# Ignaciagothe/tda-eeg-audio

Hardware: AMD Instinct MI355X
Metric: windows/sec end-to-end (dist->Rips H0/H1->Wasserstein), 47-ch EEG (higher is better)
Workload: dtype f64; 1 GPU; configs[4]+configs[2]: 1416 recordings x 5 bands x 15 selected windows = 106200 (EEG 47x250 f64, audio 250 f64) window pairs per pass, the whole job; per pair corr->dist->Rips H0/H1 (EEG 47 pts), tau per recording-band, Takens dim 3 sub 2 + Rips (audio, 23..123 pts over the bands), Wasserstein H0+H1, features, per-recording reductions; one all-gather of the (1416, 5x48) rows per pass; windows_per_pass=106200, windows_per_gpu_per_pass=106200, input_bytes_per_gpu=10195200000, batches_per_pass=1, windows_per_batch=106200, parallelism=recordings dealt over 1 rank(s), one all-gather per pass, batches_in_flight=3, hip_graph=True, batches_rerun_with_full_ladder=0

## Files before the change

### tda_eeg_audio_amd/csrc/rips.hip

```cpp
#include "common.h"
#include "corr_dist_dev.h"
#include <stdlib.h>

#ifndef CLOUD_NB
#define CLOUD_NB 8192
#endif
#ifndef NARROW_NT
#define NARROW_NT 512
#endif
#ifndef NARROW_WAVES
#define NARROW_WAVES 6
#endif
#if defined(TDA_PROFILE) && !defined(TDA_PROFILE_STOPS_ONLY)
#define NARROW_NB (NARROW_NT == 384 ? 1536 : 1024)
#else
#define NARROW_NB (NARROW_NT == 384 ? 1536 : 2048)
#endif
#define NARROW_EMAX 7626
#define NT_MAX 512
#define RANK_NONE 0x7fffu

#ifdef TDA_PROFILE
__device__ unsigned long long g_prof[48];
#ifdef TDA_PROFILE_STOPS_ONLY
#define PROF_BEGIN() do {} while (0)
#define PROF_RESUME() do {} while (0)
#define PROF_MARK(i) do {} while (0)
#define PROF_COUNT(i, v) do {} while (0)
#define PROF_FLUSH() do {} while (0)
#else
__shared__ unsigned long long prof_lds[48];
#define PROF_BEGIN()                                                       \
    if (threadIdx.x < 48) prof_lds[threadIdx.x] = 0ull;                    \
    __syncthreads();                                                       \
    unsigned long long prof_t0 = clock64()
#define PROF_RESUME() unsigned long long prof_t0 = clock64()
#define PROF_MARK(i)                                                       \
    do {                                                                   \
        unsigned long long prof_t1 = clock64();                            \
        if (threadIdx.x == 0) prof_lds[i] += prof_t1 - prof_t0;            \
        prof_t0 = prof_t1;                                                 \
// ... 95 lines not shown

__device__ __forceinline__ int edge_row(int e)
{
    const int a = (int)((1.0f + __builtin_amdgcn_sqrtf(1.0f + 8.0f * (float)e)) * 0.5f);
    const int t = tri2(a);
    return a + (t + a <= e ? 1 : 0) - (t > e ? 1 : 0);
}

#ifndef TDA_NO_EDGE_TABLE
struct EdgeTable {
    u16 v[8192 + 512];
    constexpr EdgeTable() : v()
    {
        int a = 1, b = 0;
        for (int e = 0; e < 8192 + 512; ++e) { v[e] = (u16)((a << 8) | b); if (++b == a) { ++a; b = 0; } }
    }
};
__device__ const EdgeTable g_edge_ab = EdgeTable();
__device__ __forceinline__ u32 edge_ab(int e) { return (u32)g_edge_ab.v[e]; }
#else
__device__ __forceinline__ u32 edge_ab(int e) { const int a = edge_row(e); return (u32)((a << 8) | (e - tri2(a))); }
#endif

struct WgVote {
    u32* slots;
    int parity;
};
template <int NT>
__device__ __forceinline__ bool wg_any(WgVote& v, bool p)
{
    static_assert(NT % 64 == 0 && NT <= 512, "slots are read as one or two 16-byte words; slots beyond NT / 64 hold zero");
    const bool w = __ballot(p) != 0ull;
    u32* s = v.slots + 8 * v.parity;
    if ((threadIdx.x & 63) == 0) s[threadIdx.x >> 6] = w ? 1u : 0u;
    __syncthreads();
    v.parity ^= 1;
    const uint4 x = *reinterpret_cast<const uint4*>(s);
    u32 r = x.x | x.y | x.z | x.w;
    if (NT > 256) { const uint4 y = *reinterpret_cast<const uint4*>(s + 4); r |= y.x | y.y | y.z | y.w; }
    return r != 0u;
}
template <int NT>
__device__ __forceinline__ bool wg_all(WgVote& v, bool p) { return !wg_any<NT>(v, !p); }

__device__ __forceinline__ int wave_incl_scan_i32(int v)
{
#define TDA_DPP_ADD_(CTRL, RM) v += __builtin_amdgcn_update_dpp(0, v, CTRL, RM, 0xF, true)
    TDA_DPP_ADD_(0x111, 0xF);
    TDA_DPP_ADD_(0x112, 0xF);
    TDA_DPP_ADD_(0x114, 0xF);
    TDA_DPP_ADD_(0x118, 0xF);
    TDA_DPP_ADD_(0x142, 0xA);
    TDA_DPP_ADD_(0x143, 0xC);
#undef TDA_DPP_ADD_
    return v;
}

// ... 289 lines not shown
    return __syncthreads_or(bad ? 1 : 0) ? TDA_WIN_LDS_GUARD : 0;
}
#else
#define GUARD_BYTES 0
__device__ __forceinline__ void guard_write(unsigned char*, const RipsLayout&) {}
__device__ __forceinline__ int guard_check(unsigned char*, const RipsLayout&) { return 0; }
#endif

#define MISC_COMP 0
#define MISC_CAND 512
#define MISC_WV (512 + 128)
#define MISC_MIN (512 + 192)
#define MISC_DONE (512 + 208)
#define MISC_SORTCNT (512 + 224)
#define MISC_SHARED (MISC_DONE + NT_MAX)
#define MISC_CKEY (MISC_SHARED + 96)
#define MISC_LIST MISC_CKEY
#define MISC_LIST_BYTES (4 * NT_MAX + 1280)
#define MISC_ADJ (MISC_LIST + MISC_LIST_BYTES)
#define MISC_ADJC (MISC_ADJ + 128 * 16)
#define MISC_BRANK (MISC_ADJC + 128 * 16)
#define MISC_BYTES(ncls) (MISC_BRANK + 8 * (ncls))

template <int NT, int NVW, int W, typename WT, bool NARROW, class KEYFN>
__device__ __forceinline__ void rips_sweep(int n, int E, int Ev, const u16* rank, const u16* ord, Psi<W, WT>* psi, int psi_bytes,
                           unsigned char* misc, KEYFN keyfn, double* h0, int h0_cap, double* h1, int h1_cap,
                           int& out_k0, int& out_k1, int& out_status)
{
    static_assert(!NARROW || W == 1, "the narrow layout is the point-cloud first pass");
    int psi_cap = 0;
    const int tid0 = threadIdx.x;
    const int lane0 = tid0 & 63, wave = uni(tid0 >> 6);
    int* brank = reinterpret_cast<int*>(misc + MISC_BRANK);
    u64* cand = reinterpret_cast<u64*>(misc + MISC_CAND);
    unsigned char* done = misc + MISC_DONE;
    SweepShared* shared = reinterpret_cast<SweepShared*>(misc + MISC_SHARED);
    u64* adj = reinterpret_cast<u64*>(misc + MISC_ADJ);
    constexpr int WB = 8 * (int)sizeof(WT);
    float* bkey = reinterpret_cast<float*>(misc + MISC_BRANK + 4 * WB * W);
    u64* adjc = reinterpret_cast<u64*>(misc + MISC_ADJC);

    if constexpr (!NARROW) for (int e = tid0; e < E; e += NT) psi[e] = pzero<W, WT>();
    for (int i = tid0; i < WB * W; i += NT) { brank[i] = -1; bkey[i] = 0.f; }
    for (int i = tid0; i < 256; i += NT) { adj[i] = 0ull; adjc[i] = 0ull; }
    if (tid0 == 0) {
        u32* lc = reinterpret_cast<u32*>(misc + MISC_MIN);
        lc[0] = 0u; lc[1] = 0xffffffffu; lc[2] = 0u;
        lc[3] = 0u;
        shared->status = 0;
    }
    if (tid0 < 16) {
        reinterpret_cast<u32*>(misc + MISC_WV)[tid0] = 0u;
        cand[tid0] = 0ull;
    }
    __syncthreads();

    WgVote vote{reinterpret_cast<u32*>(misc + MISC_WV), 0};
    WT alive[W];
#pragma unroll
    for (int c = 0; c < W; ++c) alive[c] = 0;
    int k0 = 0, k1 = 0, merges = 0, status = 0;
    int compA = lane0, compB = lane0 + 64;

    int clen = NT;
    int ordcls = 0;
    int cov_next = tid0;
#ifdef TDA_PROFILE
    int prof_rneed = 0, prof_chunk = -1;
#endif
    PROF_RESUME();
    for (int r0 = 0; r0 < Ev && !status; r0 += clen) {
        int tid = tid0;
        LAUNDER(tid);
        const int lane = tid & 63;
        clen = NT;
        PROF_MARK(15);
#ifdef TDA_PROFILE
        ++prof_chunk;
#endif
        PROF_COUNT(23, 1);
        const int r = r0 + tid;
        const bool valid = r < Ev;
        int a = 1, b = 0;
        if (valid) { const u32 pk = ord[r]; a = (int)(pk >> 8); b = (int)(pk & 255u); }
        const int tab = tri2(a) + b;
        const int slot = NARROW ? r : tab;
        if constexpr (NARROW) {
            psi_cap = (psi_bytes - 2 * (E - r0)) >> 2;
            if (r < psi_cap) psi[r] = pzero<W, WT>();
        }
        u64 M[NVW], M0[NVW];
        u64 Aj[NVW], Bj[NVW];
#pragma unroll
        for (int w = 0; w < NVW; ++w) { M[w] = 0; M0[w] = 0; Aj[w] = 0; Bj[w] = 0; }
        if (valid) {
#pragma unroll
            for (int w = 0; w < NVW; ++w) { Aj[w] = adj[2 * a + w]; Bj[w] = adj[2 * b + w]; M0[w] = Aj[w] & Bj[w]; }
        }
        {
            volatile u32* turn = reinterpret_cast<volatile u32*>(misc + MISC_MIN) + 2;
            if (wave > 0) {
                int trips = 0;
                for (;;) {
                    const u32 t = (u32)uni((int)*turn);
                    if (t >= (u32)wave) break;
                    if (++trips > TDA_POLL_LIMIT) { if (lane == 0) turn[1] = 1u; break; }
                    if (t + 1u < (u32)wave) __builtin_amdgcn_s_sleep(TDA_TURN_SLEEP); else __builtin_amdgcn_s_sleep(0);
                }
            }
            __builtin_amdgcn_fence(__ATOMIC_ACQUIRE, "workgroup");
            if (valid) {
#pragma unroll
                for (int w = 0; w < NVW; ++w) M[w] = (Aj[w] | adjc[2 * a + w]) & (Bj[w] | adjc[2 * b + w]);
                atomicOr(reinterpret_cast<unsigned long long*>(&adjc[2 * a + (b >> 6)]), 1ull << (b & 63));
                atomicOr(reinterpret_cast<unsigned long long*>(&adjc[2 * b + (a >> 6)]), 1ull << (a & 63));
            }
            LDS_ORDER();
            if (lane == 0 && !(TDA_FAULT(1) && wave == 3)) *turn = (u32)wave + 1u;
        }
        if (valid) {
            const int ta0 = tri2(a), tb0 = tri2(b);
#pragma unroll
            for (int w = 0; w < NVW; ++w) {
                u64 cc = (Aj[w] | adjc[2 * a + w]) & (Bj[w] | adjc[2 * b + w]) & ~M[w];
                while (cc) {
                    const int v0 = 64 * w + __builtin_ctzll(cc); cc &= cc - 1ull;
                    const bool ok1 = cc != 0ull; const int v1 = ok1 ? 64 * w + __builtin_ctzll(cc) : v0; cc &= cc - 1ull;
                    const int t0 = tri2(v0), t1 = tri2(v1);
                    const u32 xa0 = rank[v0 < a ? ta0 + v0 : t0 + a], xb0 = rank[v0 < b ? tb0 + v0 : t0 + b];
                    const u32 xa1 = rank[v1 < a ? ta0 + v1 : t1 + a], xb1 = rank[v1 < b ? tb0 + v1 : t1 + b];
                    if ((int)(xa0 > xb0 ? xa0 : xb0) < r) M[w] |= 1ull << (v0 & 63);
                    if (ok1 && (int)(xa1 > xb1 ? xa1 : xb1) < r) M[w] |= 1ull << (v1 & 63);
                }
            }
        }
        u64 many = 0;
#pragma unroll
        for (int w = 0; w < NVW; ++w) many |= M[w];
        const bool is_cand = valid && many == 0;
        int vstar = 0, d1 = 0, d2 = 0, q1 = 0, q2 = 0;
        {
            u64 many0 = 0;
#pragma unroll
            for (int w = 0; w < NVW; ++w) many0 |= M0[w];
            if (many0) {
                if (NVW == 1 || M0[0]) vstar = __builtin_ctzll(M0[0]);
                else vstar = 64 + __builtin_ctzll(M0[NVW - 1]);
            } else if (many) {
                if (NVW == 1 || M[0]) vstar = __builtin_ctzll(M[0]);
                else vstar = 64 + __builtin_ctzll(M[NVW - 1]);
            }
            if (valid && many != 0) {
                d1 = pair_index(a, vstar); d2 = pair_index(b, vstar);
                q1 = (int)rank[d1] - r0; q2 = (int)rank[d2] - r0;
                if (TDA_FAULT(2) && tid == 77 && q1 >= 0) q1 = tid;
            }
        }
        PROF_MARK(4);
        PROF_STOPC(11, out_k0 = k0; out_k1 = k1; out_status = 0);
        u64* mbal = reinterpret_cast<u64*>(misc + MISC_COMP);
        u64* zbal = mbal + 8;
        int* offs = reinterpret_cast<int*>(mbal + 16);
        u16* freebits = reinterpret_cast<u16*>(misc + MISC_CKEY);
        float mykey = 0.f;
        if (is_cand) mykey = keyfn(r, a, b);
        {
            const u64 bal = __ballot(is_cand), zb = __ballot(is_cand && mykey == 0.0f);
            if (lane == 0) { cand[wave] = bal; zbal[wave] = zb; }
        }
        done[tid] = 0;
        __syncthreads();
        PROF_MARK(21);
        PROF_STOPC(12, out_k0 = k0; out_k1 = k1; out_status = 0);
        int nfree = 0;
#pragma unroll
        for (int c = 0; c < W; ++c) nfree += __builtin_popcountll((u64)(WT)~alive[c]);
        int ncand = 0;
#pragma unroll
        for (int w = 0; w < NT / 64; ++w) ncand += __builtin_popcountll(cand[w]);
        int btot = 0;
        if (ncand > 0) {
// ... 152 lines not shown
        bool row = mrg && mykey != 0.0f;
        const u64 below = (1ull << lane) - 1ull;
        const int bpre = offs[wave] + __builtin_popcountll(__ballot(birth) & below);
        const int rpre = offs[8 + wave] + __builtin_popcountll(__ballot(row) & below);
        btot = uni(offs[16]);
        const int rtot = uni(offs[17]), mtot = uni(offs[18]);
        if (!status) {
            if (row) {
                const int pos = k0 + rpre;
                if (pos < h0_cap) { h0[2 * pos] = 0.0; h0[2 * pos + 1] = (double)mykey; }
            }
            k0 += rtot; merges += mtot;
            if (birth) {
                const int idx = (int)freebits[bpre];
                const int cw = idx / WB, bit = idx & (WB - 1);
                Psi<W, WT> nv = pzero<W, WT>();
#pragma unroll
                for (int c = 0; c < W; ++c)
                    if (c == cw) nv.w[c] = ((WT)1 << bit);
                if (!NARROW || r < psi_cap) psi[slot] = nv;
                brank[idx] = r;
                bkey[idx] = mykey;
            }
            if (W == 1 && wave == 0 && btot > 0) {
                const int nal = __builtin_popcountll((u64)alive[0]);
                if (lane >= nal && lane < nal + btot) ordcls = (int)freebits[lane - nal];
            }
            int left = btot;
#pragma unroll
            for (int c = 0; c < W; ++c) {
                const u64 f_ = (u64)(WT)~alive[c];
                const int pc = __builtin_popcountll(f_);
                if (left >= pc) { alive[c] = (WT)~(WT)0; left -= pc; }
                else if (left > 0) {
                    int lo = 0, hi = 63;
                    while (lo < hi) {
                        const int mid = (lo + hi) >> 1;
                        if (__builtin_popcountll(f_ & ((2ull << mid) - 1ull)) >= left) hi = mid; else lo = mid + 1;
                    }
                    alive[c] |= (WT)(f_ & ((2ull << lo) - 1ull));
                    left = 0;
                }
            }
        }
        }
        if (status) break;
        PROF_MARK(5);
// ... 194 lines not shown
                const u32 wmin = wave_min_u32_dpp(firstkey);
                if (lane == 0 && wmin != 0xffffffffu) atomicMin(&lcnt[1], wmin);
            }
            __syncthreads();
            PROF_MARK(17);
            PROF_STOPC(17, out_k0 = k0; out_k1 = k1; out_status = 0);
            const u32 cnt = (u32)uni((int)lcnt[0]);
            if (cnt == 0u) break;
            const bool complete = cnt <= (u32)LCAP;
            PROF_COUNT(11, 1);
            PROF_COUNT(12, cnt);
            if (!complete) {
                PROF_COUNT(13, 1);
                if (firstkey == lcnt[1]) {
                    *reinterpret_cast<u32*>(list) = firstkey;
#pragma unroll
                    for (int c = 0; c < W; ++c) *reinterpret_cast<WT*>(list + 4 + c * (int)sizeof(WT)) = firsty.w[c];
                }
                __syncthreads();
            }
            WT alive_before[W];
#pragma unroll
            for (int c = 0; c < W; ++c) alive_before[c] = alive[c];
            if (wave == 0) {
                TDA_SOLO_BEGIN();
                const int nl = complete ? (int)cnt : 1;
                u32 ek[LPL];
                Psi<W, WT> ev[LPL];
#pragma unroll
                for (int q = 0; q < LPL; ++q) {
                    const int idx = lane + 64 * q;
                    ek[q] = 0xffffffffu; ev[q] = pzero<W, WT>();
                    if (idx < nl) {
                        ek[q] = *reinterpret_cast<const u32*>(list + ES * idx);
#pragma unroll
                        for (int c = 0; c < W; ++c)
                            ev[q].w[c] = *reinterpret_cast<const WT*>(list + ES * idx + 4 + c * (int)sizeof(WT));
                    }
                }
                if (SORTED && complete) {
                    constexpr int HW = HISTN / 256;
                    u32* hw = reinterpret_cast<u32*>(hist) + HW * lane;
                    const u32 x0 = hw[0], x1 = HW == 2 ? hw[HW - 1] : 0u;
                    const u32 s0 = __builtin_amdgcn_sad_u8(x0, 0u, 0u);
                    const u32 tot = HW == 2 ? __builtin_amdgcn_sad_u8(x1, 0u, s0) : s0;
                    const u32 before = (u32)wave_incl_scan_i32((int)tot) - tot;
                    hw[0] = x0 * 0x01010101u - x0 + before * 0x01010101u;
// ... 163 lines not shown
                    for (int c = 0; c < W; ++c)
                        if (c == ycw) alive[c] &= (WT)~((WT)1 << ybit);
                    ++nk;
                }
                PROF_MARK(31);
                PROF_COUNT(10, nk);
                if (FTAB) {
                    const bool mine_ok = lane < nk;
                    float key = 0.f;
                    if (mine_ok) {
                        const u32 pkk = ord[(int)myrk];
                        key = keyfn((int)myrk, (int)(pkk >> 8), (int)(pkk & 255u));
                    }
                    const bool emit = mine_ok && key > mybirth;
                    const u64 bal = __ballot(emit);
                    const int pos = k1 + __builtin_popcountll(bal & ((1ull << lane) - 1ull));
                    if (emit && pos < h1_cap) { h1[2 * pos] = (double)mybirth; h1[2 * pos + 1] = (double)key; }
                    k1 += __builtin_popcountll(bal);
                    if (mine_ok) {
                        Psi<W, WT>* ftab = reinterpret_cast<Psi<W, WT>*>(list);
                        ftab[WB * (int)(mycode >> 8) + (int)(mycode & 255u)] = vimg;
                    }
                }
                if (lane == 0) {
#pragma unroll
                    for (int c = 0; c < W; ++c) shared->alive[c] = (u64)alive[c];
                    shared->k1 = k1; shared->nk = nk; shared->more = more; shared->status = status;
                }
                TDA_SOLO_END();
            }
            __syncthreads();
            PROF_MARK(18);
            PROF_STOPC(18, out_k0 = k0; out_k1 = k1; out_status = 0);
            WT kmask[W];
#pragma unroll
            for (int c = 0; c < W; ++c) {
                const WT na = sizeof(WT) == 8 ? (WT)uni64(shared->alive[c]) : (WT)uni((int)(u32)shared->alive[c]);
                kmask[c] = alive_before[c] & (WT)~na; alive[c] = na;
            }
            k1 = uni(shared->k1);
            const int nk = uni(shared->nk);
            const bool more = uni(shared->more) != 0;
            status = uni(shared->status);
            if (status) break;
            if (FTAB) {
                const Psi<W, WT>* ftab = reinterpret_cast<const Psi<W, WT>*>(list);
                const int seen_end = r0 + clen < Ev ? r0 + clen : Ev;
#pragma unroll 4
                for (int rr = tid; rr < seen_end; rr += NT) {
                    const int e = NARROW ? rr : edge_flat(ord[rr]);
                    const Psi<W, WT> p = psi[e];
                    WT anyh = 0;
#pragma unroll
                    for (int c = 0; c < W; ++c) anyh |= p.w[c] & kmask[c];
                    if (!anyh) continue;
                    Psi<W, WT> q;
#pragma unroll
                    for (int c = 0; c < W; ++c) q.w[c] = p.w[c] & (WT)~kmask[c];
#pragma unroll
                    for (int c = 0; c < W; ++c) {
                        u64 hh = (u64)(p.w[c] & kmask[c]);
                        while (hh) {
                            const int bit = __builtin_ctzll(hh);
                            hh &= hh - 1ull;
                            q = pxor(q, ftab[WB * c + bit]);
                        }
                    }
// ... 9 lines not shown
                        kc[j] = j0 + j < nk ? *reinterpret_cast<const u32*>(list + ES * jj) : 0xffffffffu;
#pragma unroll
                        for (int c = 0; c < W; ++c) kw[j].w[c] = *reinterpret_cast<const WT*>(list + ES * jj + 4 + c * (int)sizeof(WT));
                    }
#pragma unroll 4
                    for (int rr = tid; rr < (r0 + clen < Ev ? r0 + clen : Ev); rr += NT) {
                        const int e = NARROW ? rr : edge_flat(ord[rr]);
                        Psi<W, WT> p = psi[e];
                        bool changed = false;
#pragma unroll
                        for (int j = 0; j < 4; ++j) {
                            if (kc[j] == 0xffffffffu) continue;
                            const int jcw = (int)(kc[j] >> 8), jbit = (int)(kc[j] & 255u);
                            WT sel = 0;
#pragma unroll
                            for (int c = 0; c < W; ++c)
                                if (c == jcw) sel = (p.w[c] >> jbit) & (WT)1;
                            if (sel) { p = pxor(p, kw[j]); changed = true; }
                        }
                        if (changed) psi[e] = p;
                    }
                }
            }
            PROF_MARK(19);
            PROF_STOPC(19, out_k0 = k0; out_k1 = k1; out_status = 0);
            if (complete && !more) break;
            if (++list_rounds > 4 * NT) { status |= TDA_WIN_CLASS_OVERFLOW; break; }
            __syncthreads();
        }
        }
        if (valid && tid < clen) {
            atomicOr(reinterpret_cast<unsigned long long*>(&adj[2 * a + (b >> 6)]), 1ull << (b & 63));
            atomicOr(reinterpret_cast<unsigned long long*>(&adj[2 * b + (a >> 6)]), 1ull << (a & 63));
        }
        if (tid < 256) adjc[tid] = 0ull;
        if (tid == 0) {
            lcnt[0] = 0u; lcnt[1] = 0xffffffffu; lcnt[2] = 0u; shared->cov_min[0] = 0x7fffffff;
            if (lcnt[3]) shared->status = TDA_WIN_NOT_CONVERGED;
        }
        __syncthreads();
        if (uni(shared->status) & TDA_WIN_NOT_CONVERGED) { status |= TDA_WIN_NOT_CONVERGED; break; }
        if (quiet) {
            int from = r0 + clen;
            int rr = (NT & (NT - 1)) == 0 ? from + ((tid - from) & (NT - 1)) : from + (((tid - from) % NT) + NT) % NT;
            rr = rr > cov_next ? rr : cov_next;
            int ru;
            for (int round = 0;; ++round) {
                PROF_COUNT(41, 1);
                bool covered = true;
                while (rr < Ev) {
                    const u32 pk = ord[rr];
                    const int ea = (int)(pk >> 8), eb = (int)(pk & 255u);
                    u64 common = adj[2 * ea] & adj[2 * eb];
                    if (NVW == 2) common |= adj[2 * ea + 1] & adj[2 * eb + 1];
                    if (common == 0ull) { covered = false; break; }
                    rr += NT;
                }
                int* cmin = &shared->cov_min[round & 1];
                {
                    const u32 wmin = wave_min_u32_dpp(covered ? 0x7fffffffu : (u32)rr);
                    if (lane == 0 && wmin != 0x7fffffffu) atomicMin(reinterpret_cast<unsigned int*>(cmin), wmin);
                }
                __syncthreads();
                ru = uni(*cmin);
// ... 9 lines not shown
                from = ru;
                __syncthreads();
                if (round == 31) break;
            }
            cov_next = rr;
            if (ru >= Ev) { PROF_COUNT(25, 1); PROF_MARK(7); break; }
            PROF_COUNT(42, 1);
            if (from > r0 + clen) {
                if constexpr (NARROW) {
                    const int cap = (psi_bytes - 2 * (E - from)) >> 2;
                    for (int r2 = r0 + clen + tid; r2 < (from < cap ? from : cap); r2 += NT) psi[r2] = pzero<W, WT>();
                    __syncthreads();
                }
                clen = from - r0;
            }
        }
        PROF_MARK(7);
        PROF_STOPC(20, out_k0 = k0; out_k1 = k1; out_status = 0);
    }
#ifdef TDA_PROFILE
    PROF_COUNT(36, prof_rneed > 4096 ? 1 : 0); PROF_COUNT(37, prof_rneed > 4608 ? 1 : 0); PROF_COUNT(38, prof_rneed > 5120 ? 1 : 0);
    PROF_COUNT(39, prof_rneed); PROF_COUNT(40, Ev);
#endif
    const int ncomp = n - merges;
    for (int i = 0; i < ncomp; ++i) {
        if (k0 < h0_cap && tid0 == 0) { h0[2 * k0] = 0.0; h0[2 * k0 + 1] = (double)INFINITY; }
        ++k0;
    }
#pragma unroll
    for (int c = 0; c < W; ++c) {
        u64 al = (u64)alive[c];
        while (al) {
            const int bit = __builtin_ctzll(al);
            al &= al - 1;
            if (k1 < h1_cap && tid0 == 0) { h1[2 * k1] = (double)bkey[WB * c + bit]; h1[2 * k1 + 1] = (double)INFINITY; }
            ++k1;
        }
    }
    if (k1 > h1_cap) status |= TDA_WIN_H1_TRUNCATED;
    out_k0 = k0; out_k1 = k1; out_status = status;
}


#define TOT_NW 128
#define TOT_SLOTS 8
#define TOT_SLOT_WORDS ((size_t)8128 * TOT_NW)
#define RETRY_GRID 512
#define RETRY_GRID_WIDE 64

template <int NT, class KEYFN>
__device__ __forceinline__ void rips_sweep_total(int n, int E, int Ev, const u16* rank, const u16* ord, float* bkey, unsigned char* misc,
                                 u64* __restrict__ psi_g, KEYFN keyfn, double* h0, int h0_cap, double* h1, int h1_cap,
                                 int& out_k0, int& out_k1, int& out_status)
{
    constexpr int NWV = NT / 64;
    const int tid = threadIdx.x, lane = tid & 63, wave = uni(tid >> 6);
    u64* adj = reinterpret_cast<u64*>(misc + MISC_ADJ);
    int* comp = reinterpret_cast<int*>(misc + MISC_COMP);
// ... 109 lines not shown
        if (tid == 0) { adj[2 * a + (b >> 6)] |= 1ull << (b & 63); adj[2 * b + (a >> 6)] |= 1ull << (a & 63); }
        __syncthreads();
    }
    int status = 0;
    const int ncomp = n - merges;
    for (int i = 0; i < ncomp; ++i) {
        if (k0 < h0_cap && tid == 0) { h0[2 * k0] = 0.0; h0[2 * k0 + 1] = (double)INFINITY; }
        ++k0;
    }
    for (int c = 0; c < nborn; ++c)
        if ((alivebit[c >> 5] >> (c & 31)) & 1u) {
            if (k1 < h1_cap && tid == 0) { h1[2 * k1] = (double)bkey[c]; h1[2 * k1 + 1] = (double)INFINITY; }
            ++k1;
        }
    if (k1 > h1_cap) status |= TDA_WIN_H1_TRUNCATED;
    out_k0 = k0; out_k1 = k1; out_status = status;
}

struct KeyFromLds {
    const u32* skey;
    __device__ __forceinline__ float operator()(int r, int, int) const { return sortable_f32(skey[r]); }
};

template <int NT, int NVW, int W, typename WT, bool TOTAL = false>
__device__ __forceinline__ void rips_dm_rest(unsigned char* smem, const int win, int n, float thresh, const u32* vmax, u32 kmin_thread,
                             const RipsLayout& L, const RipsOut& out, u64* psi_g = nullptr)
{
    const int tid = threadIdx.x;
    const int E = tri2(n);
    u32* key32 = reinterpret_cast<u32*>(smem);
    u16* members = reinterpret_cast<u16*>(smem + L.off_members);
    Psi<W, WT>* psi = reinterpret_cast<Psi<W, WT>*>(smem);
    u16* rank = reinterpret_cast<u16*>(smem + L.off_rank);
    u16* ord = reinterpret_cast<u16*>(smem + L.off_ord);
    u32* skey = reinterpret_cast<u32*>(smem + L.off_aux);
    unsigned char* misc = smem + L.off_misc;
    u32* red = reinterpret_cast<u32*>(misc + MISC_MIN);
    u32* cursor = reinterpret_cast<u32*>(misc + MISC_SORTCNT);
    int* wsum = reinterpret_cast<int*>(misc + MISC_WV);
    const u32 tkey = f32_sortable(thresh);
    u32 teff, kmin;
    PROF_RESUME();
    effective_threshold<NT>(n, tkey, vmax, kmin_thread, red, teff, kmin);
    PROF_STOP(1, if (tid == 0) { out.h0_cnt[win] = 0; out.h1_cnt[win] = 0; out.status[win] = 0; });
    const int Ev = rank_edges<NT, (NVW == 1 ? 2048 : 8192), true>(key32, E, teff, kmin, members, cursor, wsum, rank, ord, skey);
    PROF_MARK(1);
    PROF_STOP(2, if (tid == 0) { out.h0_cnt[win] = 0; out.h1_cnt[win] = 0; out.status[win] = 0; });
    guard_write(smem, L);
    int k0, k1, st;
    KeyFromLds kf{skey};
    if constexpr (TOTAL)
        rips_sweep_total<NT>(n, E, Ev, rank, ord, reinterpret_cast<float*>(smem), misc, psi_g, kf,
                             out.h0 + (size_t)win * out.h0_cap * 2, out.h0_cap,
                             out.h1 + (size_t)win * out.h1_cap * 2, out.h1_cap, k0, k1, st);
    else
    rips_sweep<NT, NVW, W, WT, false>(n, E, Ev, rank, ord, psi, 0, misc, kf,
                       out.h0 + (size_t)win * out.h0_cap * 2, out.h0_cap,
                       out.h1 + (size_t)win * out.h1_cap * 2, out.h1_cap, k0, k1, st);
    st |= guard_check(smem, L);
    PROF_MARK(3);
    PROF_COUNT(8, 1);
    PROF_COUNT(9, E);
    PROF_FLUSH();
    if (tid == 0) { out.h0_cnt[win] = k0; out.h1_cnt[win] = k1; out.status[win] = st; }
}

template <int NT, int NVW, int W, typename WT, bool TOTAL = false>
__device__ __forceinline__ void rips_dm_window(unsigned char* smem, const int win, const double* __restrict__ dm, int n, float thresh,
                               int symmetrise, const RipsLayout& L, const RipsOut& out, u64* psi_g = nullptr)
{
    const int tid = threadIdx.x;
    const int E = tri2(n);
    u32* key32 = reinterpret_cast<u32*>(smem);
    unsigned char* misc = smem + L.off_misc;
    PROF_BEGIN();
    const double* D = dm + (size_t)win * n * n;
    u32* vmax = reinterpret_cast<u32*>(misc + MISC_COMP);
    if (tid < 128) vmax[tid] = 0u;
    __syncthreads();
    u32 kmin_thread = 0xffffffffu;
    for (int e = tid; e < E; e += NT) {
        const int a = edge_row(e), b = e - tri2(a);
        double v;
        if (symmetrise) {
            v = (D[(size_t)a * n + b] + D[(size_t)b * n + a]) / 2.0;
            if (v < 0.0) v = 0.0;
        } else {
// ... 228 lines not shown
        const int a = (int)(ab >> 8), b = (int)(ab & 255u);
        const u32 sk = f32_sortable(kft(0, a, b));
        key32[e] = sk;
        kmin_thread = sk < kmin_thread ? sk : kmin_thread;
        atomicMax(&vmax[b], sk);
    }
    __syncthreads();
    row_maxima<NT>(key32, vmax, P);
    __syncthreads();
    u32 teff, kmin;
    effective_threshold<NT>(P, tkey, vmax, kmin_thread, red, teff, kmin);
    PROF_MARK(0);
    PROF_STOP(1, if (tid == 0) { out.h0_cnt[win] = 0; out.h1_cnt[win] = 0; out.status[win] = 0; });
    int Ev;
    if constexpr (NARROW) {
        ord = reinterpret_cast<u16*>(smem + NL::PSI + NL::REGION) - E;
        Ev = rank_edges_narrow<NT, NARROW_NB>(key32, E, teff, kmin, members, cursor, wsum, rank, ord);
    }
    else Ev = rank_edges<NT, CLOUD_NB, false>(key32, E, teff, kmin, members, cursor, wsum, rank, ord, nullptr);
    PROF_MARK(1);
    PROF_STOP(2, if (tid == 0) { out.h0_cnt[win] = 0; out.h1_cnt[win] = 0; out.status[win] = 0; });
    guard_write(smem, L);
    int k0, k1, st;
    if constexpr (TOTAL)
        rips_sweep_total<NT>(P, E, Ev, rank, ord, reinterpret_cast<float*>(smem), misc, psi_g, kf, h0, out.h0_cap, h1, out.h1_cap, k0, k1, st);
    else if (P <= 64)
        rips_sweep<NT, 1, W, WT, NARROW>(P, E, Ev, rank, ord, psi, NL::REGION, misc, kf, h0, out.h0_cap, h1, out.h1_cap, k0, k1, st);
    else
        rips_sweep<NT, 2, W, WT, NARROW>(P, E, Ev, rank, ord, psi, NL::REGION, misc, kf, h0, out.h0_cap, h1, out.h1_cap, k0, k1, st);
    st |= guard_check(smem, L);
    PROF_MARK(3);
    PROF_COUNT(8, 1);
    PROF_COUNT(9, E);
    PROF_FLUSH();
#ifdef TDA_DEBUG_PTS
    __syncthreads();
    for (int idx = tid; idx < P * dim; idx += NT) g_dbg[1024 + idx] = pts[idx];
#endif
    if (tid == 0) { out.h0_cnt[win] = k0; out.h1_cnt[win] = k1; out.status[win] = st; }
}

#ifndef CLOUD_WAVES
#define CLOUD_WAVES 4
#endif
template <int NT, int W, typename WT, bool RETRY, bool NARROW = false>
__global__ void __launch_bounds__(NT, RETRY ? 2 : (NARROW ? NARROW_WAVES : CLOUD_WAVES))
rips_cloud_kernel(const double* __restrict__ src, const int* __restrict__ tau_or_npts, int n_win,
                  int n_t_or_pcap, int dim, int subsample, int mode, int normalise, float thresh,
                  RipsLayout L, int p_max, int* __restrict__ n_points, RipsOut out,
                  unsigned long long* __restrict__ span, unsigned long long* __restrict__ retry_ctr)
{
    extern __shared__ __attribute__((aligned(16))) unsigned char smem[];
    if (span && blockIdx.x == 0 && threadIdx.x == 0)
        atomicExch(&span[0], wall_clock64());
    if constexpr (!RETRY) {
        if ((int)blockIdx.x < n_win)
            rips_cloud_window<NT, W, WT, NARROW>(smem, (int)blockIdx.x, src, tau_or_npts, n_t_or_pcap, dim, subsample, mode,
                                                 normalise, thresh, L, p_max, n_points, out);
    } else {
        RETRY_SCAN_BEGIN(NT, out, n_win)
            if (retry_ctr && threadIdx.x == 0) atomicAdd(retry_ctr + 1, 1ull);
            rips_cloud_window<NT, W, WT, false>(smem, win, src, tau_or_npts, n_t_or_pcap, dim, subsample, mode, normalise,
// ... 35 lines not shown
    RETRY_SCAN_BEGIN(NT, out, n_win)
        if (retry_ctr && threadIdx.x == 0) atomicAdd(retry_ctr + 2, 1ull);
        rips_cloud_window<NT, 1, u32, false, true>(smem, win, src, tau_or_npts, n_t_or_pcap, dim, subsample, mode, normalise,
                                                   thresh, L, p_max, n_points, out, psi_g);
    RETRY_SCAN_END()
}

struct WindowSource {
    const double* base; long long win_stride, group_stride; int ld, wins_per_group; const int* sel;
    __device__ __forceinline__ const double* at(int w) const
    {
        const int g = sel ? sel[w] : w;
        const int r = g / wins_per_group, k = g - r * wins_per_group;
        return base + (size_t)r * (size_t)group_stride + (size_t)k * (size_t)win_stride;
    }
    __device__ __forceinline__ int ld_of(int) const { return ld; }
};
struct RaggedWindowSource {
    const double* base; const long long* start; const long long* ld;
    __device__ __forceinline__ const double* at(int w) const { return base + start[w]; }
    __device__ __forceinline__ int ld_of(int w) const { return (int)ld[w]; }
};

template <int NB, bool RES, int W, typename WT, class SRC>
__device__ __forceinline__ void eeg_one_window(unsigned char* smem, const SRC& src, int w, int n_ch,
                                               int n_t, float thresh, const RipsLayout& L, const RipsOut& out,
                                               double* __restrict__ dist, double* __restrict__ corr)
{
    const int tid = threadIdx.x, l = tid & 63, wv = tid >> 6;
    PROF_BEGIN();
    cd_window_products<NB, RES>(smem, src.at(w), n_ch, n_t, src.ld_of(w));
    const double* accs = reinterpret_cast<const double*>(smem) + CdLayout<NB>::TILE;
    const double* sdev = accs + CdLayout<NB>::ACCS + CdLayout<NB>::CP;
    const double fact = 1.0 / (double)(n_t - 1);
    auto dist_at = [&](int i, int j, double* r_out) {
        double r = (accs[CdLayout<NB>::acc_index(i, j)] * fact / sdev[i]) / sdev[j];
        r = r > 1.0 ? 1.0 : r; r = r < -1.0 ? -1.0 : r; if (r != r) r = 0.0;
        if (r_out) *r_out = r;
        double d = sqrt_rn(2.0 * (1.0 - r));
        if (!(d > 0.0) || i == j) d = 0.0;
        return d;
    };
    const int E = tri2(n_ch);
    u32* key32 = reinterpret_cast<u32*>(smem);
    u32* vmax = reinterpret_cast<u32*>(smem + 4 * ((E + 3) & ~3));
    if (tid < 128) vmax[tid] = 0u;
    __syncthreads();
// ... 1 lines not shown
    for (int e = tid; e < E; e += 256) {
        const int a = edge_row(e), b = e - tri2(a);
        double v = (dist_at(a, b, nullptr) + dist_at(b, a, nullptr)) / 2.0;
        if (v < 0.0) v = 0.0;
        const u32 sk = f32_sortable((float)v);
        key32[e] = sk;
        kmin_thread = sk < kmin_thread ? sk : kmin_thread;
        atomicMax(&vmax[a], sk);
        atomicMax(&vmax[b], sk);
    }
    if (dist) {
        double* Dw = dist + (size_t)w * n_ch * n_ch;
        double* Cw = corr ? corr + (size_t)w * n_ch * n_ch : nullptr;
        for (int i = wv; i < n_ch; i += 4)
            if (l < n_ch) {
                double r;
                const double d = dist_at(i, l, &r);
                Dw[i * n_ch + l] = d;
                if (Cw) Cw[i * n_ch + l] = r;
            }
    }
    __syncthreads();
    PROF_MARK(0);
    rips_dm_rest<256, 1, W, WT>(smem, w, n_ch, thresh, vmax, kmin_thread, L, out);
}

#ifndef TDA_EEG_WIDE_WAVES
#define TDA_EEG_WIDE_WAVES 2
#endif
template <int NB, bool RES, int W, bool RETRY, typename WT>
#ifndef TDA_EEG_WAVES
#define TDA_EEG_WAVES 6
#endif
__global__ void __launch_bounds__(256, (W > 2 || RETRY) ? TDA_EEG_WIDE_WAVES : (RES ? 3 : TDA_EEG_WAVES))
eeg_window_kernel(WindowSource windows, int n_win, int n_ch, int n_t, float thresh, RipsLayout L, RipsOut out,
                  double* __restrict__ dist, double* __restrict__ corr, unsigned long long* __restrict__ retry_ctr)
{
    extern __shared__ __attribute__((aligned(16))) unsigned char smem[];
    if constexpr (!RETRY) {
        if ((int)blockIdx.x < n_win)
            eeg_one_window<NB, RES, W, WT>(smem, windows, (int)blockIdx.x, n_ch, n_t, thresh, L, out, dist, corr);
    } else {
        RETRY_SCAN_BEGIN(256, out, n_win)
            if (retry_ctr && threadIdx.x == 0) atomicAdd(retry_ctr, 1ull);
            eeg_one_window<NB, RES, W, WT>(smem, windows, win, n_ch, n_t, thresh, L, out, dist, corr);
        RETRY_SCAN_END()
    }
}
template <int NB, bool RES, int W, bool RETRY, typename WT>
__global__ void __launch_bounds__(256, (W > 2 || RETRY) ? TDA_EEG_WIDE_WAVES : (RES ? 3 : TDA_EEG_WAVES))
eeg_window_ragged_kernel(RaggedWindowSource windows, int n_win, int n_ch, int n_t, float thresh, RipsLayout L, RipsOut out,
                         double* __restrict__ dist, double* __restrict__ corr, unsigned long long* __restrict__ retry_ctr)
{
    extern __shared__ __attribute__((aligned(16))) unsigned char smem[];
    if constexpr (!RETRY) {
        if ((int)blockIdx.x < n_win)
            eeg_one_window<NB, RES, W, WT>(smem, windows, (int)blockIdx.x, n_ch, n_t, thresh, L, out, dist, corr);
    } else {
        RETRY_SCAN_BEGIN(256, out, n_win)
            if (retry_ctr && threadIdx.x == 0) atomicAdd(retry_ctr, 1ull);
            eeg_one_window<NB, RES, W, WT>(smem, windows, win, n_ch, n_t, thresh, L, out, dist, corr);
        RETRY_SCAN_END()
    }
}
template <int NB, bool RES, int W, bool RETRY, typename WT>
static auto eeg_kernel_of(const WindowSource*) { return eeg_window_kernel<NB, RES, W, RETRY, WT>; }
template <int NB, bool RES, int W, bool RETRY, typename WT>
static auto eeg_kernel_of(const RaggedWindowSource*) { return eeg_window_ragged_kernel<NB, RES, W, RETRY, WT>; }

static inline int align16(int x) { return (x + 15) & ~15; }

tda_status retry_lists_reserve(tda_ctx* ctx, int n_win)
{
    if (n_win <= ctx->retry_cap) return TDA_OK;
    const int cap = (n_win + 1023) & ~1023;
    const size_t one = (size_t)cap + 4;
    for (int i = 0; i < TDA_RETRY_SLOTS; ++i) {
        int* q = nullptr;
        TDA_HIP(ctx, hipMalloc((void**)&q, 3 * one * sizeof(int)));
        for (int l = 0; l < 3; ++l)
            TDA_HIP(ctx, hipMemset(q + l * one, 0, 4 * sizeof(int)));
        if (ctx->retry_buf[i]) ctx->retired.push_back(ctx->retry_buf[i]);
        ctx->retry_buf[i] = q; ctx->fin_list[i] = q + one; ctx->ws_list[i] = q + 2 * one;
    }
// ... 360 lines not shown
```

Before: 4.470 million windows/s.

## Overlap next chunk's clique-mask phase with reduction on rotated reducing wave

Adds a rotated sweep mode, on by default for the audio point-cloud narrow path. The serial reduction now runs on the last wave instead of wave 0, and when a chunk completes in one round the other waves join the chunk and compute the next chunk's masks (phase A) while the reducing wave works. The aim is to hide the serial per-chunk mask and join cost behind the single-wave reduction. In exchange it adds code complexity, a new class-overflow status path that may send more windows to the retry ladder, and tid recomputation tricks to keep register pressure down.

```diff
diff --git a/tda_eeg_audio_amd/csrc/rips.hip b/tda_eeg_audio_amd/csrc/rips.hip
--- a/tda_eeg_audio_amd/csrc/rips.hip
+++ b/tda_eeg_audio_amd/csrc/rips.hip
@@ -17,6 +17,12 @@
 #define NARROW_NB (NARROW_NT == 384 ? 1536 : 2048)
 #endif
 #define NARROW_EMAX 7626
+#ifndef TDA_ROT_AUDIO
+#define TDA_ROT_AUDIO 1
+#endif
+#ifndef TDA_ROT_EEG
+#define TDA_ROT_EEG 0
+#endif
 #define NT_MAX 512
 #define RANK_NONE 0x7fffu
 
@@ -158,6 +164,13 @@
 __device__ __forceinline__ u32 edge_ab(int e) { const int a = edge_row(e); return (u32)((a << 8) | (e - tri2(a))); }
 #endif
 
+__device__ __forceinline__ int tid_from_wave(int wave)
+{
+    u32 ones = ~0u;
+    asm volatile("" : "+s"(ones));
+    return (wave << 6) + (int)__builtin_amdgcn_mbcnt_hi(ones, __builtin_amdgcn_mbcnt_lo(ones, 0u));
+}
+
 struct WgVote {
     u32* slots;
     int parity;
@@ -168,7 +181,7 @@
     static_assert(NT % 64 == 0 && NT <= 512, "slots are read as one or two 16-byte words; slots beyond NT / 64 hold zero");
     const bool w = __ballot(p) != 0ull;
     u32* s = v.slots + 8 * v.parity;
-    if ((threadIdx.x & 63) == 0) s[threadIdx.x >> 6] = w ? 1u : 0u;
+    if (tid_from_wave(0) == 0) s[uni((int)(threadIdx.x >> 6))] = w ? 1u : 0u;
     __syncthreads();
     v.parity ^= 1;
     const uint4 x = *reinterpret_cast<const uint4*>(s);
@@ -504,15 +517,19 @@
 #define MISC_BRANK (MISC_ADJC + 128 * 16)
 #define MISC_BYTES(ncls) (MISC_BRANK + 8 * (ncls))
 
-template <int NT, int NVW, int W, typename WT, bool NARROW, class KEYFN>
+template <int NT, int NVW, int W, typename WT, bool NARROW, bool ROT, class KEYFN>
 __device__ __forceinline__ void rips_sweep(int n, int E, int Ev, const u16* rank, const u16* ord, Psi<W, WT>* psi, int psi_bytes,
                            unsigned char* misc, KEYFN keyfn, double* h0, int h0_cap, double* h1, int h1_cap,
                            int& out_k0, int& out_k1, int& out_status)
 {
     static_assert(!NARROW || W == 1, "the narrow layout is the point-cloud first pass");
+    static_assert(!ROT || W == 1, "the rotated loop keeps the class order on the reducing wave: one class word");
+    constexpr int RW = ROT ? NT / 64 - 1 : 0;
     int psi_cap = 0;
-    const int tid0 = threadIdx.x;
+    int tid0 = threadIdx.x;
+    LAUNDER(tid0);
     const int lane0 = tid0 & 63, wave = uni(tid0 >> 6);
+    auto fresh_tid = [&]() __attribute__((always_inline)) { return tid_from_wave(wave); };
     int* brank = reinterpret_cast<int*>(misc + MISC_BRANK);
     u64* cand = reinterpret_cast<u64*>(misc + MISC_CAND);
     unsigned char* done = misc + MISC_DONE;
@@ -550,28 +567,17 @@
 #ifdef TDA_PROFILE
     int prof_rneed = 0, prof_chunk = -1;
 #endif
-    PROF_RESUME();
-    for (int r0 = 0; r0 < Ev && !status; r0 += clen) {
-        int tid = tid0;
-        LAUNDER(tid);
+    bool valid = false;
+    int a = 1, b = 0;
+    u64 M[NVW];
+    int vstar = 0, d1 = 0, d2 = 0, q1 = 0, q2 = 0;
+    auto phase_a = [&](const int r0, const int tid) __attribute__((always_inline)) {
         const int lane = tid & 63;
-        clen = NT;
-        PROF_MARK(15);
-#ifdef TDA_PROFILE
-        ++prof_chunk;
-#endif
-        PROF_COUNT(23, 1);
         const int r = r0 + tid;
-        const bool valid = r < Ev;
-        int a = 1, b = 0;
+        valid = r < Ev;
+        a = 1; b = 0;
         if (valid) { const u32 pk = ord[r]; a = (int)(pk >> 8); b = (int)(pk & 255u); }
-        const int tab = tri2(a) + b;
-        const int slot = NARROW ? r : tab;
-        if constexpr (NARROW) {
-            psi_cap = (psi_bytes - 2 * (E - r0)) >> 2;
-            if (r < psi_cap) psi[r] = pzero<W, WT>();
-        }
-        u64 M[NVW], M0[NVW];
+        u64 M0[NVW];
         u64 Aj[NVW], Bj[NVW];
 #pragma unroll
         for (int w = 0; w < NVW; ++w) { M[w] = 0; M0[w] = 0; Aj[w] = 0; Bj[w] = 0; }
@@ -598,7 +604,9 @@
                 atomicOr(reinterpret_cast<unsigned long long*>(&adjc[2 * b + (a >> 6)]), 1ull << (a & 63));
             }
             LDS_ORDER();
-            if (lane == 0 && !(TDA_FAULT(1) && wave == 3)) *turn = (u32)wave + 1u;
+            u32 mine = (u32)wave;
+            LAUNDER(mine);
+            if (lane == 0 && !(TDA_FAULT(1) && wave == 3)) *turn = mine + 1u;
         }
         if (valid) {
             const int ta0 = tri2(a), tb0 = tri2(b);
@@ -619,8 +627,7 @@
         u64 many = 0;
 #pragma unroll
         for (int w = 0; w < NVW; ++w) many |= M[w];
-        const bool is_cand = valid && many == 0;
-        int vstar = 0, d1 = 0, d2 = 0, q1 = 0, q2 = 0;
+        vstar = 0; d1 = 0; d2 = 0; q1 = 0; q2 = 0;
         {
             u64 many0 = 0;
 #pragma unroll
@@ -638,7 +645,57 @@
                 if (TDA_FAULT(2) && tid == 77 && q1 >= 0) q1 = tid;
             }
         }
-        PROF_MARK(4);
+    };
+    auto join_chunk = [&](const int tid, const bool header) __attribute__((always_inline)) {
+        u32* lcnt = reinterpret_cast<u32*>(misc + MISC_MIN);
+        if (valid && tid < clen) {
+            atomicOr(reinterpret_cast<unsigned long long*>(&adj[2 * a + (b >> 6)]), 1ull << (b & 63));
+            atomicOr(reinterpret_cast<unsigned long long*>(&adj[2 * b + (a >> 6)]), 1ull << (a & 63));
+        }
+        u32 zero = 0u;
+        LAUNDER(zero);
+        if (tid < 256) adjc[tid] = (u64)zero;
+        if (tid == 0) {
+            if (header) { lcnt[0] = zero; lcnt[1] = ~zero; }
+            lcnt[2] = zero; shared->cov_min[0] = 0x7fffffff;
+            if (lcnt[3]) shared->status = TDA_WIN_NOT_CONVERGED;
+        }
+        __syncthreads();
+        return (uni(shared->status) & TDA_WIN_NOT_CONVERGED) != 0;
+    };
+    bool masks_ready = false;
+    PROF_RESUME();
+    for (int r0 = 0; r0 < Ev && !status; r0 += clen) {
+        const int tid = fresh_tid();
+        const int lane = tid & 63;
+        clen = NT;
+        PROF_MARK(15);
+#ifdef TDA_PROFILE
+        ++prof_chunk;
+#endif
+        PROF_COUNT(23, 1);
+        const int r = r0 + tid;
+        if constexpr (NARROW) {
+            psi_cap = (psi_bytes - 2 * (E - r0)) >> 2;
+            if (r < psi_cap) psi[r] = pzero<W, WT>();
+        }
+        if (!ROT || !masks_ready) {
+            phase_a(r0, tid);
+            PROF_MARK(4);
+        }
+        masks_ready = false;
+        if constexpr (ROT) {
+            valid = r < Ev;
+            a = 1; b = 0;
+            if (valid) { const u32 pk = ord[r]; a = (int)(pk >> 8); b = (int)(pk & 255u); }
+        }
+        u64 many = 0;
+#pragma unroll
+        for (int w = 0; w < NVW; ++w) many |= M[w];
+        const int tab = tri2(a) + b;
+        const int slot = NARROW ? r : tab;
+        const bool is_cand = valid && many == 0;
+        bool joined = false;
         PROF_STOPC(11, out_k0 = k0; out_k1 = k1; out_status = 0);
         u64* mbal = reinterpret_cast<u64*>(misc + MISC_COMP);
         u64* zbal = mbal + 8;
@@ -837,7 +894,7 @@
                 brank[idx] = r;
                 bkey[idx] = mykey;
             }
-            if (W == 1 && wave == 0 && btot > 0) {
+            if (W == 1 && wave == RW && btot > 0) {
                 const int nal = __builtin_popcountll((u64)alive[0]);
                 if (lane >= nal && lane < nal + btot) ordcls = (int)freebits[lane - nal];
             }
@@ -1078,7 +1135,18 @@
             WT alive_before[W];
 #pragma unroll
             for (int c = 0; c < W; ++c) alive_before[c] = alive[c];
-            if (wave == 0) {
+            bool overlap = false;
+            if constexpr (ROT) {
+                overlap = complete && r0 + clen < Ev;
+                if (overlap) {
+                    joined = true;
+                    if (join_chunk(tid, false)) { status |= TDA_WIN_NOT_CONVERGED; break; }
+                    if (tid == 0) { lcnt[0] = 0u; lcnt[1] = 0xffffffffu; }
+                    PROF_MARK(46);
+                    PROF_COUNT(45, 1);
+                }
+            }
+            if (wave == RW) {
                 TDA_SOLO_BEGIN();
                 const int nl = complete ? (int)cnt : 1;
                 u32 ek[LPL];
@@ -1288,6 +1356,7 @@
                         ftab[WB * (int)(mycode >> 8) + (int)(mycode & 255u)] = vimg;
                     }
                 }
+                if (ROT && more) status |= TDA_WIN_CLASS_OVERFLOW;
                 if (lane == 0) {
 #pragma unroll
                     for (int c = 0; c < W; ++c) shared->alive[c] = (u64)alive[c];
@@ -1295,20 +1364,22 @@
                 }
                 TDA_SOLO_END();
             }
+            WT kmask[W];
+            int nk = 0;
+            bool more = false;
+            auto round_end = [&]() __attribute__((always_inline)) {
             __syncthreads();
-            PROF_MARK(18);
-            PROF_STOPC(18, out_k0 = k0; out_k1 = k1; out_status = 0);
-            WT kmask[W];
 #pragma unroll
             for (int c = 0; c < W; ++c) {
                 const WT na = sizeof(WT) == 8 ? (WT)uni64(shared->alive[c]) : (WT)uni((int)(u32)shared->alive[c]);
                 kmask[c] = alive_before[c] & (WT)~na; alive[c] = na;
             }
             k1 = uni(shared->k1);
-            const int nk = uni(shared->nk);
-            const bool more = uni(shared->more) != 0;
+            nk = uni(shared->nk);
+            more = uni(shared->more) != 0;
             status = uni(shared->status);
-            if (status) break;
+            };
+            auto rewrite = [&]() __attribute__((always_inline)) {
             if (FTAB) {
                 const Psi<W, WT>* ftab = reinterpret_cast<const Psi<W, WT>*>(list);
                 const int seen_end = r0 + clen < Ev ? r0 + clen : Ev;
@@ -1364,6 +1435,25 @@
                     }
                 }
             }
+            };
+            if constexpr (ROT) {
+                if (overlap) {
+                    phase_a(r0 + clen, tid);
+                    masks_ready = true;
+                    PROF_MARK(43);
+                    round_end();
+                    PROF_MARK(44);
+                    if (status) break;
+                    rewrite();
+                    PROF_MARK(19);
+                    break;
+                }
+            }
+            round_end();
+            PROF_MARK(18);
+            PROF_STOPC(18, out_k0 = k0; out_k1 = k1; out_status = 0);
+            if (status) break;
+            rewrite();
             PROF_MARK(19);
             PROF_STOPC(19, out_k0 = k0; out_k1 = k1; out_status = 0);
             if (complete && !more) break;
@@ -1371,17 +1461,10 @@
             __syncthreads();
         }
         }
-        if (valid && tid < clen) {
-            atomicOr(reinterpret_cast<unsigned long long*>(&adj[2 * a + (b >> 6)]), 1ull << (b & 63));
-            atomicOr(reinterpret_cast<unsigned long long*>(&adj[2 * b + (a >> 6)]), 1ull << (a & 63));
-        }
-        if (tid < 256) adjc[tid] = 0ull;
-        if (tid == 0) {
-            lcnt[0] = 0u; lcnt[1] = 0xffffffffu; lcnt[2] = 0u; shared->cov_min[0] = 0x7fffffff;
-            if (lcnt[3]) shared->status = TDA_WIN_NOT_CONVERGED;
-        }
-        __syncthreads();
-        if (uni(shared->status) & TDA_WIN_NOT_CONVERGED) { status |= TDA_WIN_NOT_CONVERGED; break; }
+        if constexpr (ROT) { if (status) break; }
+        if (!ROT || !joined) {
+            if (join_chunk(tid, true)) { status |= TDA_WIN_NOT_CONVERGED; break; }
+        }
         if (quiet) {
             int from = r0 + clen;
             int rr = (NT & (NT - 1)) == 0 ? from + ((tid - from) & (NT - 1)) : from + (((tid - from) % NT) + NT) % NT;
@@ -1437,9 +1520,10 @@
     PROF_COUNT(36, prof_rneed > 4096 ? 1 : 0); PROF_COUNT(37, prof_rneed > 4608 ? 1 : 0); PROF_COUNT(38, prof_rneed > 5120 ? 1 : 0);
     PROF_COUNT(39, prof_rneed); PROF_COUNT(40, Ev);
 #endif
+    const int tid_end = fresh_tid();
     const int ncomp = n - merges;
     for (int i = 0; i < ncomp; ++i) {
-        if (k0 < h0_cap && tid0 == 0) { h0[2 * k0] = 0.0; h0[2 * k0 + 1] = (double)INFINITY; }
+        if (k0 < h0_cap && tid_end == 0) { h0[2 * k0] = 0.0; h0[2 * k0 + 1] = (double)INFINITY; }
         ++k0;
     }
 #pragma unroll
@@ -1448,7 +1532,7 @@
         while (al) {
             const int bit = __builtin_ctzll(al);
             al &= al - 1;
-            if (k1 < h1_cap && tid0 == 0) { h1[2 * k1] = (double)bkey[WB * c + bit]; h1[2 * k1 + 1] = (double)INFINITY; }
+            if (k1 < h1_cap && tid_end == 0) { h1[2 * k1] = (double)bkey[WB * c + bit]; h1[2 * k1 + 1] = (double)INFINITY; }
             ++k1;
         }
     }
@@ -1604,7 +1688,7 @@
     __device__ __forceinline__ float operator()(int r, int, int) const { return sortable_f32(skey[r]); }
 };
 
-template <int NT, int NVW, int W, typename WT, bool TOTAL = false>
+template <int NT, int NVW, int W, typename WT, bool TOTAL = false, bool ROT = false>
 __device__ __forceinline__ void rips_dm_rest(unsigned char* smem, const int win, int n, float thresh, const u32* vmax, u32 kmin_thread,
                              const RipsLayout& L, const RipsOut& out, u64* psi_g = nullptr)
 {
@@ -1630,13 +1714,14 @@
     PROF_STOP(2, if (tid == 0) { out.h0_cnt[win] = 0; out.h1_cnt[win] = 0; out.status[win] = 0; });
     guard_write(smem, L);
     int k0, k1, st;
+    const int wave_s = uni(tid >> 6);
     KeyFromLds kf{skey};
     if constexpr (TOTAL)
         rips_sweep_total<NT>(n, E, Ev, rank, ord, reinterpret_cast<float*>(smem), misc, psi_g, kf,
                              out.h0 + (size_t)win * out.h0_cap * 2, out.h0_cap,
                              out.h1 + (size_t)win * out.h1_cap * 2, out.h1_cap, k0, k1, st);
     else
-    rips_sweep<NT, NVW, W, WT, false>(n, E, Ev, rank, ord, psi, 0, misc, kf,
+    rips_sweep<NT, NVW, W, WT, false, ROT>(n, E, Ev, rank, ord, psi, 0, misc, kf,
                        out.h0 + (size_t)win * out.h0_cap * 2, out.h0_cap,
                        out.h1 + (size_t)win * out.h1_cap * 2, out.h1_cap, k0, k1, st);
     st |= guard_check(smem, L);
@@ -1644,7 +1729,7 @@
     PROF_COUNT(8, 1);
     PROF_COUNT(9, E);
     PROF_FLUSH();
-    if (tid == 0) { out.h0_cnt[win] = k0; out.h1_cnt[win] = k1; out.status[win] = st; }
+    if (tid_from_wave(wave_s) == 0) { out.h0_cnt[win] = k0; out.h1_cnt[win] = k1; out.status[win] = st; }
 }
 
 template <int NT, int NVW, int W, typename WT, bool TOTAL = false>
@@ -1919,12 +2004,13 @@
     PROF_STOP(2, if (tid == 0) { out.h0_cnt[win] = 0; out.h1_cnt[win] = 0; out.status[win] = 0; });
     guard_write(smem, L);
     int k0, k1, st;
+    const int wave_s = uni(tid >> 6);
     if constexpr (TOTAL)
         rips_sweep_total<NT>(P, E, Ev, rank, ord, reinterpret_cast<float*>(smem), misc, psi_g, kf, h0, out.h0_cap, h1, out.h1_cap, k0, k1, st);
     else if (P <= 64)
-        rips_sweep<NT, 1, W, WT, NARROW>(P, E, Ev, rank, ord, psi, NL::REGION, misc, kf, h0, out.h0_cap, h1, out.h1_cap, k0, k1, st);
+        rips_sweep<NT, 1, W, WT, NARROW, NARROW && TDA_ROT_AUDIO>(P, E, Ev, rank, ord, psi, NL::REGION, misc, kf, h0, out.h0_cap, h1, out.h1_cap, k0, k1, st);
     else
-        rips_sweep<NT, 2, W, WT, NARROW>(P, E, Ev, rank, ord, psi, NL::REGION, misc, kf, h0, out.h0_cap, h1, out.h1_cap, k0, k1, st);
+        rips_sweep<NT, 2, W, WT, NARROW, NARROW && TDA_ROT_AUDIO>(P, E, Ev, rank, ord, psi, NL::REGION, misc, kf, h0, out.h0_cap, h1, out.h1_cap, k0, k1, st);
     st |= guard_check(smem, L);
     PROF_MARK(3);
     PROF_COUNT(8, 1);
@@ -1934,7 +2020,7 @@
     __syncthreads();
     for (int idx = tid; idx < P * dim; idx += NT) g_dbg[1024 + idx] = pts[idx];
 #endif
-    if (tid == 0) { out.h0_cnt[win] = k0; out.h1_cnt[win] = k1; out.status[win] = st; }
+    if (tid_from_wave(wave_s) == 0) { out.h0_cnt[win] = k0; out.h1_cnt[win] = k1; out.status[win] = st; }
 }
 
 #ifndef CLOUD_WAVES
@@ -2016,7 +2102,7 @@
     __device__ __forceinline__ int ld_of(int w) const { return (int)ld[w]; }
 };
 
-template <int NB, bool RES, int W, typename WT, class SRC>
+template <int NB, bool RES, int W, typename WT, bool ROT, class SRC>
 __device__ __forceinline__ void eeg_one_window(unsigned char* smem, const SRC& src, int w, int n_ch,
                                                int n_t, float thresh, const RipsLayout& L, const RipsOut& out,
                                                double* __restrict__ dist, double* __restrict__ corr)
@@ -2064,7 +2150,7 @@
     }
     __syncthreads();
     PROF_MARK(0);
-    rips_dm_rest<256, 1, W, WT>(smem, w, n_ch, thresh, vmax, kmin_thread, L, out);
+    rips_dm_rest<256, 1, W, WT, false, ROT>(smem, w, n_ch, thresh, vmax, kmin_thread, L, out);
 }
 
 #ifndef TDA_EEG_WIDE_WAVES
@@ -2081,11 +2167,11 @@
     extern __shared__ __attribute__((aligned(16))) unsigned char smem[];
     if constexpr (!RETRY) {
         if ((int)blockIdx.x < n_win)
-            eeg_one_window<NB, RES, W, WT>(smem, windows, (int)blockIdx.x, n_ch, n_t, thresh, L, out, dist, corr);
+            eeg_one_window<NB, RES, W, WT, W == 1 && TDA_ROT_EEG>(smem, windows, (int)blockIdx.x, n_ch, n_t, thresh, L, out, dist, corr);
     } else {
         RETRY_SCAN_BEGIN(256, out, n_win)
             if (retry_ctr && threadIdx.x == 0) atomicAdd(retry_ctr, 1ull);
-            eeg_one_window<NB, RES, W, WT>(smem, windows, win, n_ch, n_t, thresh, L, out, dist, corr);
+            eeg_one_window<NB, RES, W, WT, false>(smem, windows, win, n_ch, n_t, thresh, L, out, dist, corr);
         RETRY_SCAN_END()
     }
 }
@@ -2097,11 +2183,11 @@
     extern __shared__ __attribute__((aligned(16))) unsigned char smem[];
     if constexpr (!RETRY) {
         if ((int)blockIdx.x < n_win)
-            eeg_one_window<NB, RES, W, WT>(smem, windows, (int)blockIdx.x, n_ch, n_t, thresh, L, out, dist, corr);
+            eeg_one_window<NB, RES, W, WT, W == 1 && TDA_ROT_EEG>(smem, windows, (int)blockIdx.x, n_ch, n_t, thresh, L, out, dist, corr);
     } else {
         RETRY_SCAN_BEGIN(256, out, n_win)
             if (retry_ctr && threadIdx.x == 0) atomicAdd(retry_ctr, 1ull);
-            eeg_one_window<NB, RES, W, WT>(smem, windows, win, n_ch, n_t, thresh, L, out, dist, corr);
+            eeg_one_window<NB, RES, W, WT, false>(smem, windows, win, n_ch, n_t, thresh, L, out, dist, corr);
         RETRY_SCAN_END()
     }
 }
```

Result: no change. 4.500 million windows/s (median of 6 runs) (+0.7%).
